# jlko/STOVE

Measured on AMD Instinct MI355X. Metric: frames/s (fwd+bwd) for 3-obj billiards 32x32 T=100, 1/2/4/8 GPU; ELBO delta vs ref, higher is better.
Workload: dtype f32 (encoder GEMMs: fp32 products as 3 sixteen-bit MFMAs on hi/lo-split operands -- half pieces forward, bf16 pieces backward -- fp32 accumulate)

## Files before the change

### stove_amd/csrc/capi.hip

```cpp
#include "../../include/stove_hip.h"
#include <algorithm>

#include "common.h"
#include <string.h>
#include <stdlib.h>
#include <math.h>
#include <atomic>
#include <type_traits>
#include "validate.h"
static_assert(stove_validate::kStoveInvalidValue == (int)hipErrorInvalidValue, "validate.h returns hipErrorInvalidValue");
#define STOVE_VALIDATE(expr)                      \
  do {                                            \
    const int v__ = stove_validate::expr;         \
    if (v__) return v__;                          \
  } while (0)
#include "spn_obj.hip"
#include "spn_obj_generic.hip"
#include "spn_bg.hip"
#include "spn_bg_generic.hip"
#include "scene.hip"
#include "scene_fused.hip"
#include "scene_colour.hip"
#include "gnn.hip"
#include "match.hip"
// ... 317 lines not shown
    inl = scene_any_inline(W_, H_);
    boxes.z = inl ? z : nullptr; boxes.n_obj = n_obj; boxes.gm = gm;
    plane = W_ * H_;
    channels = channels_;
  }
  int fork() {
    sb = scene_fork_stream(st);
    STOVE_TRY(stream_after(sb, root));
    jb.from = sb; jb.done = sb == st;
    jp.from = sp; jp.done = sp == st;
    return 0;
  }
};

template <class Obj, class Bg>
static int scene_forward(SceneCall& c, float overlap_beta, float* ll, float* parts, Obj obj_chain, Bg bg_chain) {
  int rc = c.fork();
  if (rc) return rc;
  if ((rc = obj_chain())) return rc;
  if ((rc = bg_chain())) return rc;
  STOVE_TRY(c.jb.join());
  STOVE_LAUNCH(scene_assemble_fwd_k, dim3((c.nf + 255) / 256), dim3(256), 0, c.st, c.saved + c.L.bg_out, c.saved + c.L.obj_ll,
               c.saved + c.L.ovl, c.z, ll, parts, c.n_obj, c.nf, overlap_beta, logf(overlap_beta));
  STOVE_LAUNCH_CHECK();
  return 0;
}

template <class Side, class Obj, class After>
static int scene_backward(SceneCall& c, const float* dll, float* dz, float overlap_beta, int nmax, const float* dz_bg, int bg_parts,
                          Side side_chains, Obj obj_chain, After after_finalize) {
  STOVE_LAUNCH(scene_assemble_bwd_k, dim3((c.np + 255) / 256), dim3(256), 0, c.st, dll, c.z, c.ws + c.W.d_obj, c.ws + c.W.d_ovl, c.n_obj,
               c.np, overlap_beta);
  STOVE_LAUNCH_CHECK();
  int rc = c.fork();
  if (rc) return rc;
  if ((rc = side_chains())) return rc;
  if ((rc = obj_chain())) return rc;
  STOVE_TRY(c.jb.join());
  rc = with_nmax(nmax, [&](auto n) {
    STOVE_LAUNCH((scene_finalize_bwd_k<decltype(n)::value>), dim3((c.np + 255) / 256), dim3(256), 0, c.st, dll, c.z, c.saved + c.L.obj_ll,
                 dz_bg, c.ws + c.W.dzc, dz, c.n_obj, c.np, bg_parts);
    STOVE_LAUNCH_CHECK();
    return 0;
  });
  if (rc) return rc;
  if ((rc = after_finalize())) return rc;
  c.jp.dismiss();
  return 0;
}

template <bool ANY>
static int scene_obj_fwd(const SceneCall& c, const StoveSpnTables* t, float* saved, int with_grad) {
  float* xw = saved + c.L.xw;
  int rc = with_nmax(c.n_obj, [&](auto n) { return scene_tile_fwd<decltype(n)::value, ANY>(c.frames, c.z, xw, c.n_obj, c.np, c.st, c.fm, c.gm); });
  if (rc) return rc;
  if (with_grad)
    return objspn_forward_unit(xw, t->obj_scope, t->obj_coef, t->obj_wsum, t->obj_wroot, saved + c.L.obj_ll, saved + c.L.ovl,
                               saved + c.L.obj_scratch, c.np, c.st);
  return objspn_forward(xw, t->obj_scope, t->obj_coef, t->obj_wsum, t->obj_wroot, saved + c.L.obj_ll, saved + c.L.ovl, c.np, c.st);
}
template <bool ANY>
static int scene_obj_bwd(const SceneCall& c, const StoveSpnTables* t) {
  return with_nmax(c.n_obj, [&](auto n) {
    return scene_pixtile_bwd<decltype(n)::value, ANY>(c.frames, c.z, c.saved + c.L.xw, c.saved + c.L.obj_scratch, t->obj_leaf_slot, t->obj_coef,
                                                      c.ws + c.W.d_ovl, c.ws + c.W.dzc, c.n_obj, c.np, c.st, c.fm, c.ws + c.W.d_obj, c.gm);
  });
}
static int scene_obj_tablegrads(const SceneCall& c, const StoveSpnTables* t, StoveSpnTableGrads* g, bool under = false) {
  STOVE_TRY(stream_after(c.sp, c.st));
  return objspn_backward_params(c.saved + c.L.xw, t->obj_scope, g->obj_coef, g->obj_wsum, g->obj_wroot, c.saved + c.L.obj_scratch,
                                c.ws + c.W.obj, c.ws + c.W.d_obj, c.np, c.sp, under);
}

static int scene_bg_fwd_any(const SceneCall& c, const int32_t* side, const float* coef, const float* wroot, float* saved) {
  if (!c.inl) {
    const size_t tot = (size_t)c.nf * c.plane;
    STOVE_LAUNCH(bg_mask_any_k, dim3((unsigned)((tot + 255) / 256)), dim3(256), 0, c.sb, c.z, saved + c.L.bg_aux, c.nf, c.n_obj, c.gm);
    STOVE_LAUNCH_CHECK();
  }
  return bgspn_any_forward(c.frames, c.inl ? nullptr : saved + c.L.bg_aux, side, coef, wroot, saved + c.L.bg_ell, saved + c.L.bg_out, c.nf,
                           c.channels * c.plane, c.sb, c.fm, c.boxes, c.plane);
}
static int scene_bg_bwd_any(const SceneCall& c, const int32_t* side, const float* coef, const float* wroot, const float* dll, float* g_coef,
                            float* g_wroot) {
  float* d_mask = c.ws + c.W.d_mask;
  int rc = bgspn_any_backward(c.frames, c.inl ? nullptr : c.saved + c.L.bg_aux, side, coef, wroot, c.saved + c.L.bg_ell, c.saved + c.L.bg_out,
                              dll, nullptr, d_mask, g_coef, g_wroot, c.ws + c.W.bg, c.nf, c.channels * c.plane, c.sb, c.fm, c.boxes, c.plane);
  if (rc) return rc;
  return with_nmax<false>(c.n_obj, [&](auto n) {
    STOVE_LAUNCH((bg_mask_bwd_any_k<decltype(n)::value>), dim3(c.nf), dim3(256), 0, c.sb, c.z, (const float*)d_mask, c.ws + c.W.dz_bg, c.nf,
                 c.n_obj, c.gm, c.channels);
    STOVE_LAUNCH_CHECK();
    return 0;
  });
}

}

extern "C" {

static SceneSaved scene_saved_tuned(int nf, int n_obj, bool with_grad = true) {
  return scene_saved_layout(nf, n_obj, with_grad, bgspn_fwd_ws_floats(nf), bg_cover_floats(nf, n_obj));
}
static SceneWs scene_ws_tuned(int nf, int n_obj) {
  return scene_ws_layout((size_t)nf * n_obj, nmax_of(n_obj), 0, objspn_partial_floats(), 0, bgspn_bwd_ws_floats(nf, n_obj));
}
size_t stove_scene_saved_floats(int n_frames, int n_obj) { return scene_saved_tuned(n_frames, n_obj).total; }
size_t stove_scene_fwd_floats(int n_frames, int n_obj, int with_grad) { return scene_saved_tuned(n_frames, n_obj, with_grad != 0).total; }
size_t stove_scene_bwd_ws_bytes(int n_frames, int n_obj) { return scene_ws_tuned(n_frames, n_obj).total * sizeof(float); }

size_t stove_bg_dense_floats(void) { return (size_t)kBgDenseF; }
int stove_bg_dense(const int32_t* bg_side, const float* bg_coef, float* dense, void* stream) {
  STOVE_LAUNCH(bg_dense_fwd_k, dim3((kBgDenseF + 255) / 256), dim3(256), 0, (hipStream_t)stream, bg_side, bg_coef, dense);
  STOVE_LAUNCH_CHECK();
  return 0;
}
int stove_scene_fwd(const StoveSpnTables* t, const float* frames, const float* z, int n_frames, int n_obj, int seq_frames,
                    int seq_stride, float overlap_beta, float* ll, float* parts, float* saved, void* stream) {
  return stove_scene_fwd_from(t, frames, z, n_frames, n_obj, seq_frames, seq_stride, overlap_beta, ll, parts, saved, stream, stream, 1);
}

int stove_scene_fwd_from(const StoveSpnTables* t, const float* frames, const float* z, int n_frames, int n_obj, int seq_frames,
                         int seq_stride, float overlap_beta, float* ll, float* parts, float* saved, void* stream, void* fork_from,
                         int with_grad) {
  STOVE_VALIDATE(scene_fwd(t, frames, z, n_frames, n_obj, seq_frames, seq_stride, ll, saved));
  if (n_frames == 0) return 0;
  SceneCall c(frames, z, n_frames, n_obj, stream, fork_from);
  if (frame_map(n_frames, seq_frames, seq_stride, &c.fm)) return (int)hipErrorInvalidValue;
  c.L = scene_saved_tuned(n_frames, n_obj);
  c.saved = saved;
  return scene_forward(
      c, overlap_beta, ll, parts, [&] { return scene_obj_fwd<false>(c, t, saved, with_grad); },
      [&] {
        int rc = bgspn_forward(frames, nullptr, z, n_obj, t->bg_side, t->bg_coef, t->bg_wroot, saved + c.L.bg_ell, saved + c.L.bg_out, n_frames,
                               c.sb, c.fm, t->bg_dense);
        if (rc) return rc;
        return bg_cover_tables(z, saved + c.L.bg_aux, n_frames, n_obj, c.sb);
      });
}

int stove_scene_bwd(const StoveSpnTables* t, const float* frames, const float* z, int n_frames, int n_obj, int seq_frames,
                    int seq_stride, float overlap_beta, const float* saved, const float* dll, float* dz, StoveSpnTableGrads* g,
                    void* ws_, void* stream) {
  return stove_scene_bwd_overlap(t, frames, z, n_frames, n_obj, seq_frames, seq_stride, overlap_beta, saved, dll, dz, g, ws_, stream, stream);
}

int stove_scene_bwd_overlap(const StoveSpnTables* t, const float* frames, const float* z, int n_frames, int n_obj, int seq_frames,
                            int seq_stride, float overlap_beta, const float* saved, const float* dll, float* dz,
                            StoveSpnTableGrads* g, void* ws_, void* stream, void* param_stream) {
  return stove_scene_bwd_from(t, frames, z, n_frames, n_obj, seq_frames, seq_stride, overlap_beta, saved, dll, dz, g, ws_, stream, param_stream, stream);
}

constexpr int kLateTableGradGlimpses = 16384;

int stove_scene_bwd_from(const StoveSpnTables* t, const float* frames, const float* z, int n_frames, int n_obj, int seq_frames,
                         int seq_stride, float overlap_beta, const float* saved, const float* dll, float* dz,
                         StoveSpnTableGrads* g, void* ws_, void* stream, void* param_stream, void* fork_from) {
  STOVE_VALIDATE(scene_bwd(t, frames, z, n_frames, n_obj, seq_frames, seq_stride, saved, dll, dz, g, ws_));
  if (n_frames == 0) return 0;
  SceneCall c(frames, z, n_frames, n_obj, stream, fork_from, param_stream);
  if (frame_map(n_frames, seq_frames, seq_stride, &c.fm)) return (int)hipErrorInvalidValue;
  c.L = scene_saved_tuned(n_frames, n_obj);
  c.saved = saved;
  c.W = scene_ws_tuned(n_frames, n_obj);
  c.ws = (float*)ws_;
  const bool late = c.sp != c.st && n_obj <= 4 && c.np >= kLateTableGradGlimpses;
  return scene_backward(
      c, dll, dz, overlap_beta, nmax_of(n_obj), bgspn_dz_parts(c.ws + c.W.bg, n_frames), kBgHalves,
      [&] {
        if (!late) {
          const int rc = scene_obj_tablegrads(c, t, g);
          if (rc) return rc;
        }
        return bgspn_backward(frames, nullptr, z, n_obj, t->bg_side, t->bg_coef, t->bg_wroot, saved + c.L.bg_ell, saved + c.L.bg_out, dll, nullptr,
                              nullptr, nullptr, g->bg_coef, g->bg_wroot, c.ws + c.W.bg, n_frames, c.sb, c.sp == c.st ? c.sb : c.sp, c.fm,
                              saved + c.L.bg_aux);
      },
      [&] { return scene_obj_bwd<false>(c, t); }, [&] { return late ? scene_obj_tablegrads(c, t, g, true) : 0; });
}

static ObjAnyShape obj_any_shape(int R, int G, int S, int D, int Lmax) {
  ObjAnyShape sh;
  sh.R = R; sh.G = G; sh.S = S; sh.D = D; sh.Lmax = Lmax;
  return sh;
}
size_t stove_objspn_saved_floats_any(int n, int R, int G, int S, int D, int Lmax) { return objany_saved_floats(n, obj_any_shape(R, G, S, D, Lmax)); }
size_t stove_objspn_bwd_ws_bytes_any(int n, int R, int G, int S, int D, int Lmax) { return objany_bwd_ws_floats(n, obj_any_shape(R, G, S, D, Lmax)) * sizeof(float); }
int stove_objspn_fwd_any(const float* inputs, const float* marg, const int* lscope, const float* coef, const float* wsum, const float* wroot,
                         float* saved, float* out, int n, int R, int G, int S, int D, int Lmax, void* stream) {
  return objany_forward(inputs, marg, lscope, coef, wsum, wroot, saved, out, n, obj_any_shape(R, G, S, D, Lmax), (hipStream_t)stream);
}
int stove_objspn_bwd_any(const float* inputs, const float* marg, const int* lscope, const int* slot, const float* coef, const float* wsum,
                         const float* wroot, const float* saved, const float* dout, float* d_inputs, float* d_marg, float* g_coef,
                         float* g_wsum, float* g_wroot, void* ws, int n, int R, int G, int S, int D, int Lmax, void* stream) {
  return objany_backward(inputs, marg, lscope, slot, coef, wsum, wroot, saved, dout, d_inputs, d_marg, g_coef, g_wsum, g_wroot, (float*)ws, n,
                         obj_any_shape(R, G, S, D, Lmax), (hipStream_t)stream);
}

int stove_gauss_ll_fwd(const float* x, const float* marg, float* out, int n, int d, float mean, float scale, void* stream) {
  if (n == 0) return 0;
  if (d < 1 || !(scale > 0.0f) || x == nullptr || marg == nullptr || out == nullptr) return (int)hipErrorInvalidValue;
  STOVE_LAUNCH(gauss_ll_fwd_k, dim3((n + 3) / 4), dim3(256), 0, (hipStream_t)stream, x, marg, out, n, d, mean, scale);
  STOVE_LAUNCH_CHECK();
  return 0;
}
int stove_gauss_ll_bwd(const float* x, const float* marg, const float* dout, float* dx, float* dm, int n, int d, float mean, float scale,
                       void* stream) {
  if (n == 0) return 0;
  if (d < 1 || !(scale > 0.0f) || x == nullptr || marg == nullptr || dout == nullptr) return (int)hipErrorInvalidValue;
  const size_t tot = (size_t)n * d;
  STOVE_LAUNCH(gauss_ll_bwd_k, dim3((unsigned)((tot + 255) / 256)), dim3(256), 0, (hipStream_t)stream, x, marg, dout, dx, dm, n, d, mean, scale);
  STOVE_LAUNCH_CHECK();
  return 0;
}

static SceneSaved scene_saved_any(int nf, int n_obj, int n_pix, bool with_grad, bool inline_mask = false) {
  return scene_saved_layout(nf, n_obj, with_grad, bgspn_any_saved_floats(nf, n_pix), inline_mask ? 0 : (size_t)nf * n_pix);
}
static SceneWs scene_ws_any(int nf, int n_obj, int n_pix) {
  return scene_ws_layout((size_t)nf * n_obj, nmax_of(n_obj), 0, objspn_partial_floats(), (size_t)nf * n_pix, bgspn_any_bwd_ws_floats(nf, n_pix));
}
size_t stove_scene_saved_floats_any(int n_frames, int n_obj, int n_pix, int with_grad) { return scene_saved_any(n_frames, n_obj, n_pix, with_grad != 0).total; }
size_t stove_scene_bwd_ws_bytes_any(int n_frames, int n_obj, int n_pix) { return scene_ws_any(n_frames, n_obj, n_pix).total * sizeof(float); }

int stove_scene_fwd_any(const StoveSpnTables* t, const float* frames, const float* z, int n_frames, int n_obj, int seq_frames, int seq_stride,
                        int W, int H, int align_corners, float overlap_beta, float* ll, float* parts, float* saved, void* stream, int with_grad) {
  STOVE_VALIDATE(scene_fwd(t, frames, z, n_frames, n_obj, seq_frames, seq_stride, ll, saved));
  if (n_frames == 0) return 0;
  if (W < 2 || H < 2 || n_obj < 1 || n_obj > 8) return (int)hipErrorInvalidValue;
  SceneCall c(frames, z, n_frames, n_obj, stream);
  if (frame_map(n_frames, seq_frames, seq_stride, &c.fm)) return (int)hipErrorInvalidValue;
  c.geometry(W, H, align_corners, 1);
  c.L = scene_saved_any(n_frames, n_obj, W * H, true, c.inl);
  c.saved = saved;
  return scene_forward(
      c, overlap_beta, ll, parts, [&] { return scene_obj_fwd<true>(c, t, saved, with_grad); },
      [&] { return scene_bg_fwd_any(c, t->bg_side, t->bg_coef, t->bg_wroot, saved); });
}

int stove_scene_bwd_any(const StoveSpnTables* t, const float* frames, const float* z, int n_frames, int n_obj, int seq_frames, int seq_stride,
                        int W, int H, int align_corners, float overlap_beta, const float* saved, const float* dll, float* dz,
                        StoveSpnTableGrads* g, void* ws_, void* stream, void* param_stream) {
  STOVE_VALIDATE(scene_bwd(t, frames, z, n_frames, n_obj, seq_frames, seq_stride, saved, dll, dz, g, ws_));
  if (n_frames == 0) return 0;
  if (W < 2 || H < 2 || n_obj < 1 || n_obj > 8) return (int)hipErrorInvalidValue;
  SceneCall c(frames, z, n_frames, n_obj, stream, nullptr, param_stream);
  if (frame_map(n_frames, seq_frames, seq_stride, &c.fm)) return (int)hipErrorInvalidValue;
  c.geometry(W, H, align_corners, 1);
  c.L = scene_saved_any(n_frames, n_obj, W * H, true, c.inl);
  c.saved = saved;
  c.W = scene_ws_any(n_frames, n_obj, W * H);
  c.ws = (float*)ws_;
  return scene_backward(
      c, dll, dz, overlap_beta, nmax_of(n_obj), c.ws + c.W.dz_bg, 1,
      [&] { return scene_bg_bwd_any(c, t->bg_side, t->bg_coef, t->bg_wroot, dll, g->bg_coef, g->bg_wroot); },
      [&] { return scene_obj_bwd<true>(c, t); },
      [&] { return scene_obj_tablegrads(c, t, g); });
}

static inline int nmax_ch(int n_obj) { return n_obj <= 3 ? 3 : 8; }
static SceneSaved scene_saved_ch(int nf, int n_obj, int C, int W, int H, const ObjAnyShape& sh) {
  const size_t np = (size_t)nf * n_obj;
  Layout l;
  SceneSaved s{};
  s.patches = l.take(np * sh.D);
  s.marg = l.take(np * sh.D);
  s.obj = l.take(objany_saved_floats((int)np, sh));
  scene_saved_shared(l, s, nf, np, bgspn_any_saved_floats(nf, C * W * H), scene_any_inline(W, H) ? 0 : (size_t)nf * W * H);
  s.total = l.total;
  return s;
}
static SceneWs scene_ws_ch(int nf, int n_obj, int C, int W, int H, const ObjAnyShape& sh) {
  const size_t np = (size_t)nf * n_obj, n_pix = (size_t)C * W * H;
  return scene_ws_layout(np, nmax_ch(n_obj), np * sh.D, objany_bwd_ws_floats((int)np, sh), (size_t)nf * n_pix, bgspn_any_bwd_ws_floats(nf, (int)n_pix));
}
static GlimpseGeom glimpse_geom(int pw, int ph, int align_corners) {
  GlimpseGeom g;
  g.pw = pw; g.ph = ph;
  if (align_corners) {
    g.pax = 2.0f / (ph - 1); g.pbx = -1.0f; g.pay = 2.0f / (pw - 1); g.pby = -1.0f;
  } else {
    g.pax = 2.0f / ph; g.pbx = 1.0f / ph - 1.0f; g.pay = 2.0f / pw; g.pby = 1.0f / pw - 1.0f;
  }
  return g;
}
size_t stove_scene_saved_floats_ch(int n_frames, int n_obj, int channels, int W, int H, int R, int G, int S, int D, int Lmax, int with_grad) {
  (void)with_grad;
  return scene_saved_ch(n_frames, n_obj, channels, W, H, obj_any_shape(R, G, S, D, Lmax)).total;
}
size_t stove_scene_bwd_ws_bytes_ch(int n_frames, int n_obj, int channels, int W, int H, int R, int G, int S, int D, int Lmax) {
  return scene_ws_ch(n_frames, n_obj, channels, W, H, obj_any_shape(R, G, S, D, Lmax)).total * sizeof(float);
}

int stove_scene_fwd_ch(const int32_t* lscope, const int32_t* slot, const float* coef, const float* wsum, const float* wroot, int R, int G, int S,
                       int D, int Lmax, const int32_t* bg_side, const float* bg_coef, const float* bg_wroot, size_t bg_coef_floats,
                       const float* frames, const float* z, int n_frames, int n_obj, int seq_frames, int seq_stride, int channels, int W, int H,
                       int pw, int ph, int align_corners, float overlap_beta, float* ll, float* parts, float* saved, void* stream, int with_grad) {
  (void)slot;
  (void)with_grad;
  STOVE_VALIDATE(scene_ch_fwd(lscope, coef, wsum, wroot, R, G, S, D, Lmax, bg_side, bg_coef, bg_wroot, bg_coef_floats, frames, z, n_frames, n_obj,
                              seq_frames, seq_stride, channels, W, H, pw, ph, ll, saved));
  if (n_frames == 0) return 0;
  SceneCall c(frames, z, n_frames, n_obj, stream);
  if (frame_map(n_frames, seq_frames, seq_stride, &c.fm)) return (int)hipErrorInvalidValue;
  const ObjAnyShape sh = obj_any_shape(R, G, S, D, Lmax);
  const GlimpseGeom gg = glimpse_geom(pw, ph, align_corners);
// ... 1466 lines not shown
```

### stove_amd/csrc/spn_obj.hip

```cpp
#include "common.h"

namespace stove {

template <int N>
__device__ __forceinline__ float vmax(const float (&v)[N]) {
  float m = v[0];
#pragma unroll
  for (int i = 1; i < N; ++i) m = fmaxf(m, v[i]);
  return m;
}

template <int N>
struct LaneTable {
  float v[(N + 63) / 64];
  __device__ __forceinline__ void load(const float* __restrict__ p, int lane) {
#pragma unroll
    for (int i = 0; i < (N + 63) / 64; ++i) v[i] = (i * 64 + lane < N) ? p[i * 64 + lane] : 0.0f;
  }
  __device__ __forceinline__ float at(int idx) const {
    return __int_as_float(__builtin_amdgcn_readlane(__float_as_int(v[idx >> 6]), idx & 63));
  }
};

template <int N>
// ... 475 lines not shown
  const float4 sc = wrow ? tg_scale4(scale, first_sample + 4 * (threadIdx.x & 15)) : float4{1.0f, 1.0f, 1.0f, 1.0f};
  for (int i = threadIdx.x; i < 2 * D * 16; i += NT) {
    float4 v = src[i];
    v.x *= sc.x; v.y *= sc.y; v.z *= sc.z; v.w *= sc.w;
    *reinterpret_cast<float4*>(tileP + (i >> 4) * LD + 4 * (i & 15)) = v;
  }
}

template <int R, int S, int G, int K>
__global__ __launch_bounds__(128 * R) void objspn_tablegrad_k(
    const float* __restrict__ xw, const float* __restrict__ Dscr, const float* __restrict__ Sscr, const float* __restrict__ Rscr,
    const int* __restrict__ scope, float* __restrict__ part_c, float* __restrict__ part_w, float* __restrict__ part_r,
    int n_batches, int n_chunks, const float* __restrict__ scale) {
  constexpr int D = 4 * S, LD = 68, NS = K + 2 * G;
  constexpr int TC = (3 * S + 15) / 16, TW = (G * G + 15) / 16;
  static_assert(G <= 16 && K <= 16, "one column tile");
  typedef __attribute__((ext_vector_type(4))) float f4;
  extern __shared__ __attribute__((aligned(16))) float tg_lds[];
  float* tileP = tg_lds;
  float* nodeS = tileP + 2 * D * LD;
  const int lane = lane_id(), wv = wave_id();
  const int r = wv >> 1, side = wv & 1, node = wv;
  const int rr = lane & 15, kk = lane >> 4;
  const int c = blockIdx.x;
  int c_row[2][TC], c_feat[2][TC];
#pragma unroll
  for (int l2 = 0; l2 < 2; ++l2)
#pragma unroll
    for (int t = 0; t < TC; ++t) {
      const int row = min(16 * t + rr, 3 * S - 1);
      c_feat[l2][t] = row / S;
      c_row[l2][t] = 2 * scope[(r * 4 + side * 2 + l2) * S + row % S];
    }
  int w_e1[TW], w_e2[TW];
#pragma unroll
  for (int t = 0; t < TW; ++t) {
    const int row = min(16 * t + rr, G * G - 1);
    w_e1[t] = K + row % G;
    w_e2[t] = K + G + row / G;
  }
  f4 acc_c[2][TC], acc_w[TW], acc_r;
#pragma unroll
  for (int l2 = 0; l2 < 2; ++l2)
#pragma unroll
    for (int t = 0; t < TC; ++t) acc_c[l2][t] = f4{0.0f, 0.0f, 0.0f, 0.0f};
#pragma unroll
  for (int t = 0; t < TW; ++t) acc_w[t] = f4{0.0f, 0.0f, 0.0f, 0.0f};
  acc_r = f4{0.0f, 0.0f, 0.0f, 0.0f};

  for (int b = c; b < n_batches; b += n_chunks) {
    {
      tg_stage_tile<D, LD, 128 * R>(tileP, xw + (size_t)b * (D * 2 * 64), scale, b * 64);
      const float4* ss = reinterpret_cast<const float4*>(Sscr + (size_t)(b * R * 2 + node) * NS * 64);
      float* dst = nodeS + node * NS * LD;
      for (int i = lane; i < NS * 16; i += 64) *reinterpret_cast<float4*>(dst + (i >> 4) * LD + 4 * (i & 15)) = ss[i];
    }
    __syncthreads();
#pragma unroll
    for (int l2 = 0; l2 < 2; ++l2) {
      const int L = side * 2 + l2;
      const float4* dp = reinterpret_cast<const float4*>(Dscr + (((size_t)(b * R + r) * 4 + L) * G + min(rr, G - 1)) * 64 + 16 * kk);
      const float4 d0 = dp[0], d1 = dp[1], d2 = dp[2], d3 = dp[3];
      const float dv[16] = {d0.x, d0.y, d0.z, d0.w, d1.x, d1.y, d1.z, d1.w, d2.x, d2.y, d2.z, d2.w, d3.x, d3.y, d3.z, d3.w};
#pragma unroll
      for (int t = 0; t < TC; ++t) {
        const float* xr = tileP + c_row[l2][t] * LD + 16 * kk;
        const int feat = c_feat[l2][t];
#pragma unroll
        for (int h = 0; h < 4; ++h) {
          const float4 x4 = *reinterpret_cast<const float4*>(xr + 4 * h);
          const float4 w4 = *reinterpret_cast<const float4*>(xr + LD + 4 * h);
          const float xs[4] = {x4.x, x4.y, x4.z, x4.w}, ws[4] = {w4.x, w4.y, w4.z, w4.w};
#pragma unroll
          for (int e = 0; e < 4; ++e) {
            const float wx = ws[e] * xs[e];
            const float fv = feat == 0 ? wx * xs[e] : (feat == 1 ? wx : ws[e]);
            acc_c[l2][t] = __builtin_amdgcn_mfma_f32_16x16x4f32(fv, dv[4 * h + e], acc_c[l2][t], 0, 0, 0);
          }
        }
      }
    }
    {
      const float* nb = nodeS + node * NS * LD + 16 * kk;
      const float* gp = nb + min(rr, K - 1) * LD;
      float gv[16];
#pragma unroll
      for (int h = 0; h < 4; ++h) {
        const float4 g4 = *reinterpret_cast<const float4*>(gp + 4 * h);
        const float4 s4 = tg_scale4(scale, b * 64 + 16 * kk + 4 * h);
        gv[4 * h] = g4.x * s4.x; gv[4 * h + 1] = g4.y * s4.y; gv[4 * h + 2] = g4.z * s4.z; gv[4 * h + 3] = g4.w * s4.w;
      }
#pragma unroll
      for (int t = 0; t < TW; ++t) {
        const float* e1 = nb + w_e1[t] * LD;
        const float* e2 = nb + w_e2[t] * LD;
#pragma unroll
        for (int h = 0; h < 4; ++h) {
          const float4 a4 = *reinterpret_cast<const float4*>(e1 + 4 * h);
          const float4 b4 = *reinterpret_cast<const float4*>(e2 + 4 * h);
          acc_w[t] = __builtin_amdgcn_mfma_f32_16x16x4f32(a4.x * b4.x, gv[4 * h], acc_w[t], 0, 0, 0);
          acc_w[t] = __builtin_amdgcn_mfma_f32_16x16x4f32(a4.y * b4.y, gv[4 * h + 1], acc_w[t], 0, 0, 0);
          acc_w[t] = __builtin_amdgcn_mfma_f32_16x16x4f32(a4.z * b4.z, gv[4 * h + 2], acc_w[t], 0, 0, 0);
          acc_w[t] = __builtin_amdgcn_mfma_f32_16x16x4f32(a4.w * b4.w, gv[4 * h + 3], acc_w[t], 0, 0, 0);
        }
      }
    }
    if (side == 0) {
      const float* rp = Rscr + (size_t)(b * R + r) * (1 + 2 * K) * 64 + 16 * kk;
      const float4* rho = reinterpret_cast<const float4*>(rp);
      const float4* ea = reinterpret_cast<const float4*>(rp + (1 + min(rr, K - 1)) * 64);
      const float4* eb = reinterpret_cast<const float4*>(rp + (1 + K + min(rr, K - 1)) * 64);
#pragma unroll
      for (int h = 0; h < 4; ++h) {
        const float4 q4 = rho[h], a4 = ea[h], b4 = eb[h];
        const float4 s4 = tg_scale4(scale, b * 64 + 16 * kk + 4 * h);
        acc_r = __builtin_amdgcn_mfma_f32_16x16x4f32(q4.x * s4.x * b4.x, a4.x, acc_r, 0, 0, 0);
        acc_r = __builtin_amdgcn_mfma_f32_16x16x4f32(q4.y * s4.y * b4.y, a4.y, acc_r, 0, 0, 0);
        acc_r = __builtin_amdgcn_mfma_f32_16x16x4f32(q4.z * s4.z * b4.z, a4.z, acc_r, 0, 0, 0);
        acc_r = __builtin_amdgcn_mfma_f32_16x16x4f32(q4.w * s4.w * b4.w, a4.w, acc_r, 0, 0, 0);
      }
    }
    __syncthreads();
  }
  const int col = lane & 15;
#pragma unroll
  for (int l2 = 0; l2 < 2; ++l2)
#pragma unroll
    for (int t = 0; t < TC; ++t)
#pragma unroll
      for (int e = 0; e < 4; ++e) {
        const int row = 16 * t + 4 * kk + e;
        if (row < 3 * S && col < G) {
          const int feat = row / S, i = row % S;
          part_c[((size_t)(c * R + r) * D + (side * 2 + l2) * S + i) * G * 3 + col * 3 + feat] = acc_c[l2][t][e];
        }
      }
#pragma unroll
  for (int t = 0; t < TW; ++t)
#pragma unroll
    for (int e = 0; e < 4; ++e) {
      const int row = 16 * t + 4 * kk + e;
      if (row < G * G && col < K) part_w[((size_t)(c * R * 2 + node) * G * G + row) * K + col] = acc_w[t][e];
    }
  if (side == 0) {
#pragma unroll
    for (int e = 0; e < 4; ++e) {
      const int row = 4 * kk + e;
      if (row < K && col < K) part_r[((size_t)(c * R + r) * K + row) * K + col] = acc_r[e];
    }
  }
}

template <int R, int S, int G, int K>
__global__ __launch_bounds__(256, 3) void objspn_tablegrad_under_k(
   
    const float* __restrict__ xw, const float* __restrict__ Dscr, const float* __restrict__ Sscr, const float* __restrict__ Rscr,
    const int* __restrict__ scope, float* __restrict__ part_c, float* __restrict__ part_w, float* __restrict__ part_r,
    int n_batches, int n_chunks, const float* __restrict__ scale) {
  constexpr int D = 4 * S, LD = 68, NS = K + 2 * G;
  constexpr int TC = (3 * S + 15) / 16, TW = (G * G + 15) / 16, TWH = (TW + 1) / 2;
  static_assert(G <= 16 && K <= 16, "one column tile");
  typedef __attribute__((ext_vector_type(4))) float f4;
  extern __shared__ __attribute__((aligned(16))) float tg_lds[];
  float* tileP = tg_lds;
  float* scl = tileP + 2 * D * LD;
  const int lane = lane_id(), wv = wave_id();
  int c, r;
  if ((n_chunks & 7) == 0) {
    const int xcd = blockIdx.x & 7, j = blockIdx.x >> 3;
    c = xcd * (n_chunks >> 3) + j / R;
    r = j % R;
  } else {
    c = blockIdx.x / R;
    r = blockIdx.x % R;
  }
  const int side = wv & 1, half = wv >> 1, node = 2 * r + side, L = side * 2 + half;
  const int rr = lane & 15, kk = lane >> 4;
  int c_row[TC], c_feat[TC];
#pragma unroll
  for (int t = 0; t < TC; ++t) {
    const int row = min(16 * t + rr, 3 * S - 1);
    c_feat[t] = row / S;
    c_row[t] = 2 * scope[(r * 4 + L) * S + row % S];
  }
  int w_e1[TWH], w_e2[TWH];
#pragma unroll
  for (int i = 0; i < TWH; ++i) {
    const int row = min(16 * (half * TWH + i) + rr, G * G - 1);
    w_e1[i] = K + row % G;
    w_e2[i] = K + G + row / G;
  }
  f4 acc_c[TC], acc_w[TWH], acc_r = f4{0.0f, 0.0f, 0.0f, 0.0f};
#pragma unroll
  for (int t = 0; t < TC; ++t) acc_c[t] = f4{0.0f, 0.0f, 0.0f, 0.0f};
#pragma unroll
  for (int i = 0; i < TWH; ++i) acc_w[i] = f4{0.0f, 0.0f, 0.0f, 0.0f};

  for (int b = c; b < n_batches; b += n_chunks) {
    tg_stage_tile<D, LD, 256>(tileP, xw + (size_t)b * (D * 2 * 64), scale, b * 64);
    if (threadIdx.x < 16) *reinterpret_cast<float4*>(scl + 4 * threadIdx.x) = tg_scale4(scale, b * 64 + 4 * threadIdx.x);
    __syncthreads();
    {
      const float4* dp = reinterpret_cast<const float4*>(Dscr + (((size_t)(b * R + r) * 4 + L) * G + min(rr, G - 1)) * 64 + 16 * kk);
      const float4 d0 = dp[0], d1 = dp[1], d2 = dp[2], d3 = dp[3];
      const float dv[16] = {d0.x, d0.y, d0.z, d0.w, d1.x, d1.y, d1.z, d1.w, d2.x, d2.y, d2.z, d2.w, d3.x, d3.y, d3.z, d3.w};
#pragma unroll
      for (int h = 0; h < 4; ++h) {
        float fv[TC][4];
#pragma unroll
        for (int t = 0; t < TC; ++t) {
          const float* xr = tileP + c_row[t] * LD + 16 * kk + 4 * h;
          const float4 x4 = *reinterpret_cast<const float4*>(xr);
          const float4 w4 = *reinterpret_cast<const float4*>(xr + LD);
          const float xs[4] = {x4.x, x4.y, x4.z, x4.w}, ws[4] = {w4.x, w4.y, w4.z, w4.w};
#pragma unroll
          for (int e = 0; e < 4; ++e) {
            const float wx = ws[e] * xs[e];
            fv[t][e] = c_feat[t] == 0 ? wx * xs[e] : (c_feat[t] == 1 ? wx : ws[e]);
          }
        }
#pragma unroll
        for (int e = 0; e < 4; ++e)
#pragma unroll
          for (int t = 0; t < TC; ++t) acc_c[t] = __builtin_amdgcn_mfma_f32_16x16x4f32(fv[t][e], dv[4 * h + e], acc_c[t], 0, 0, 0);
      }
    }
    {
      const float* nb = Sscr + (size_t)(b * R * 2 + node) * NS * 64 + 16 * kk;
      const float* gp = nb + min(rr, K - 1) * 64;
#pragma unroll
      for (int h = 0; h < 4; ++h) {
        const float4 g4 = *reinterpret_cast<const float4*>(gp + 4 * h);
        const float4 s4 = *reinterpret_cast<const float4*>(scl + 16 * kk + 4 * h);
        const float gv[4] = {g4.x * s4.x, g4.y * s4.y, g4.z * s4.z, g4.w * s4.w};
        float pr[TWH][4];
#pragma unroll
        for (int i = 0; i < TWH; ++i) {
          const float4 a4 = *reinterpret_cast<const float4*>(nb + w_e1[i] * 64 + 4 * h);
          const float4 b4 = *reinterpret_cast<const float4*>(nb + w_e2[i] * 64 + 4 * h);
          pr[i][0] = a4.x * b4.x; pr[i][1] = a4.y * b4.y; pr[i][2] = a4.z * b4.z; pr[i][3] = a4.w * b4.w;
        }
#pragma unroll
        for (int e = 0; e < 4; ++e)
#pragma unroll
          for (int i = 0; i < TWH; ++i)
            acc_w[i] = __builtin_amdgcn_mfma_f32_16x16x4f32(pr[i][e], gv[e], acc_w[i], 0, 0, 0);
      }
    }
    if (side == 0 && half == 1) {
      const float* rp = Rscr + (size_t)(b * R + r) * (1 + 2 * K) * 64 + 16 * kk;
      const float4* rho = reinterpret_cast<const float4*>(rp);
      const float4* ea = reinterpret_cast<const float4*>(rp + (1 + min(rr, K - 1)) * 64);
      const float4* eb = reinterpret_cast<const float4*>(rp + (1 + K + min(rr, K - 1)) * 64);
#pragma unroll
      for (int h = 0; h < 4; ++h) {
        const float4 q4 = rho[h], a4 = ea[h], b4 = eb[h];
        const float4 s4 = *reinterpret_cast<const float4*>(scl + 16 * kk + 4 * h);
        acc_r = __builtin_amdgcn_mfma_f32_16x16x4f32(q4.x * s4.x * b4.x, a4.x, acc_r, 0, 0, 0);
        acc_r = __builtin_amdgcn_mfma_f32_16x16x4f32(q4.y * s4.y * b4.y, a4.y, acc_r, 0, 0, 0);
        acc_r = __builtin_amdgcn_mfma_f32_16x16x4f32(q4.z * s4.z * b4.z, a4.z, acc_r, 0, 0, 0);
        acc_r = __builtin_amdgcn_mfma_f32_16x16x4f32(q4.w * s4.w * b4.w, a4.w, acc_r, 0, 0, 0);
      }
    }
    __syncthreads();
  }
  const int col = lane & 15;
#pragma unroll
  for (int t = 0; t < TC; ++t)
#pragma unroll
    for (int e = 0; e < 4; ++e) {
      const int row = 16 * t + 4 * kk + e;
      if (row < 3 * S && col < G) {
        const int feat = row / S, i = row % S;
        part_c[((size_t)(c * R + r) * D + L * S + i) * G * 3 + col * 3 + feat] = acc_c[t][e];
      }
    }
#pragma unroll
  for (int i = 0; i < TWH; ++i)
#pragma unroll
    for (int e = 0; e < 4; ++e) {
      const int row = 16 * (half * TWH + i) + 4 * kk + e;
      if (row < G * G && col < K) part_w[((size_t)(c * R * 2 + node) * G * G + row) * K + col] = acc_w[i][e];
    }
  if (side == 0 && half == 1) {
#pragma unroll
    for (int e = 0; e < 4; ++e) {
      const int row = 4 * kk + e;
      if (row < K && col < K) part_r[((size_t)(c * R + r) * K + row) * K + col] = acc_r[e];
    }
  }
}

__global__ void objspn_tile_from_arrays_k(const float* __restrict__ inputs, const float* __restrict__ marg,
                                          float* __restrict__ xw, int n_samples, int n_batches, int D) {
  extern __shared__ float lds[];
  const int stride = D + 1;
  for (int b = blockIdx.x; b < n_batches; b += gridDim.x) {
    for (int i = threadIdx.x; i < 64 * D; i += blockDim.x) {
      const int smp = i / D, p = i % D;
      const size_t gi = (size_t)(b * 64 + smp) * D + p;
      const bool live = (b * 64 + smp) < n_samples;
      const float x = live ? inputs[gi] : 0.0f;
      float w = 0.0f;
      if (live) w = (marg != nullptr) ? 1.0f - fminf(fmaxf(marg[gi], 0.0f), 1.0f) : 1.0f;
      lds[smp * stride + p] = x;
      lds[64 * stride + smp * stride + p] = w;
    }
    __syncthreads();
    float* tile = xw + (size_t)b * D * 2 * 64;
    for (int i = threadIdx.x; i < 64 * D * 2; i += blockDim.x) {
      const int lane = i & 63, pc = i >> 6;
      tile[i] = lds[(pc & 1) * 64 * stride + lane * stride + (pc >> 1)];
    }
    __syncthreads();
  }
}

__global__ void objspn_tile_to_arrays_k(const float* __restrict__ dxw, const float* __restrict__ marg,
                                        float* __restrict__ d_inputs, float* __restrict__ d_marg,
                                        int n_samples, int n_batches, int D) {
  extern __shared__ float lds[];
  const int stride = D + 1;
  for (int b = blockIdx.x; b < n_batches; b += gridDim.x) {
    const float* tile = dxw + (size_t)b * D * 2 * 64;
    for (int i = threadIdx.x; i < 64 * D * 2; i += blockDim.x) {
      const int lane = i & 63, pc = i >> 6;
      lds[(pc & 1) * 64 * stride + lane * stride + (pc >> 1)] = tile[i];
    }
    __syncthreads();
    for (int i = threadIdx.x; i < 64 * D; i += blockDim.x) {
      const int smp = i / D, p = i % D;
      if ((b * 64 + smp) >= n_samples) continue;
      const size_t gi = (size_t)(b * 64 + smp) * D + p;
      if (d_inputs != nullptr) d_inputs[gi] = lds[smp * stride + p];
      if (d_marg != nullptr) {
        const float m = marg[gi];
        d_marg[gi] = (m >= 0.0f && m <= 1.0f) ? -lds[64 * stride + smp * stride + p] : 0.0f;
      }
    }
    __syncthreads();
  }
}

__global__ __launch_bounds__(256) void reduce_chunks_k(const float* __restrict__ part, float* __restrict__ out, int n, int n_chunks, int accumulate,
                                                       float* __restrict__ out2 = nullptr) {
  __shared__ float red[8][32];
  const int e = threadIdx.x & 31, q = threadIdx.x >> 5;
  const int j = blockIdx.x * 32 + e;
  float s = 0.0f;
  if (j < n)
    for (int c = q; c < n_chunks; c += 8) s += part[(size_t)c * n + j];
  red[q][e] = s;
  __syncthreads();
  if (q == 0 && j < n) {
    float t = red[0][e];
#pragma unroll
    for (int k = 1; k < 8; ++k) t += red[k][e];
    out[j] = accumulate ? out[j] + t : t;
    if (out2 != nullptr) out2[j] = accumulate ? out2[j] + t : t;
  }
}

struct Reduce3 {
  const float* part[3];
  float* out[3];
  int n[3];
};
__global__ __launch_bounds__(256) void reduce_chunks3_k(Reduce3 a, int n_chunks) {
  __shared__ float red[8][32];
  const int e = threadIdx.x & 31, q = threadIdx.x >> 5;
  int blk = blockIdx.x, seg = 0;
#pragma unroll
  for (int k = 0; k < 2; ++k) {
    const int nbk = (a.n[k] + 31) / 32;
    if (seg == k && blk >= nbk) {
      blk -= nbk;
      seg = k + 1;
    }
  }
  const float* __restrict__ part = seg == 0 ? a.part[0] : (seg == 1 ? a.part[1] : a.part[2]);
  float* __restrict__ out = seg == 0 ? a.out[0] : (seg == 1 ? a.out[1] : a.out[2]);
  const int n = seg == 0 ? a.n[0] : (seg == 1 ? a.n[1] : a.n[2]);
  const int j = blk * 32 + e;
  float s = 0.0f;
  if (j < n)
    for (int c = q; c < n_chunks; c += 8) s += part[(size_t)c * n + j];
  red[q][e] = s;
  __syncthreads();
  if (q == 0 && j < n) {
    float t = red[0][e];
#pragma unroll
    for (int k = 1; k < 8; ++k) t += red[k][e];
    out[j] = t;
  }
}

}

namespace stove {

static inline int grid_for(int n_items, int cap) { return n_items < cap ? (n_items > 0 ? n_items : 1) : cap; }

int objspn_tile_from_arrays(const float* inputs, const float* marg, float* xw, int n, hipStream_t st) {
  const int nb = (n + 63) / 64;
  if (nb == 0) return 0;
  const int D = 100;
  STOVE_LAUNCH(objspn_tile_from_arrays_k, dim3(grid_for(nb, 2048)), dim3(256), 2 * 64 * (D + 1) * sizeof(float), st,
                     inputs, marg, xw, n, nb, D);
  STOVE_LAUNCH_CHECK();
  return 0;
}

int objspn_tile_to_arrays(const float* dxw, const float* marg, float* d_inputs, float* d_marg, int n, hipStream_t st) {
  const int nb = (n + 63) / 64;
  if (nb == 0) return 0;
  const int D = 100;
  STOVE_LAUNCH(objspn_tile_to_arrays_k, dim3(grid_for(nb, 2048)), dim3(256), 2 * 64 * (D + 1) * sizeof(float), st,
                     dxw, marg, d_inputs, d_marg, n, nb, D);
  STOVE_LAUNCH_CHECK();
  return 0;
}

int objspn_forward(const float* xw, const int* scope, const float* coef, const float* wsum, const float* wroot,
                   float* out, float* ovl, int n, hipStream_t st) {
  const int nb = (n + 63) / 64;
  if (nb == 0) return 0;
  STOVE_LAUNCH((objspn_fwd_k<6, 25, 10, 10>), dim3(grid_for(nb, 4096)), dim3(768), 0, st,
                     xw, scope, coef, wsum, wroot, out, ovl, n, nb);
  STOVE_LAUNCH_CHECK();
  return 0;
}

int objspn_mpe(const float* xw, const int* scope, const float* coef, const float* wsum, const float* wroot, const float* mu,
               float* out, int* pick, int n, hipStream_t st) {
  const int nb = (n + 63) / 64;
  if (nb == 0) return 0;
  STOVE_LAUNCH((objspn_mpe_k<6, 25, 10, 10>), dim3(grid_for(nb, 4096)), dim3(768), 0, st,
                     xw, scope, coef, wsum, wroot, mu, out, pick, n, nb);
  STOVE_LAUNCH_CHECK();
  return 0;
}

constexpr size_t kObjD = 6 * 4 * 10 * 64, kObjS = 12 * 30 * 64, kObjR = 6 * 21 * 64, kObjX = 100 * 2 * 64;
constexpr int kObjChunks = 256;
constexpr size_t kObjCoefN = 6 * 100 * 10 * 3, kObjWN = 12 * 100 * 10, kObjRootN = 6 * 100;

size_t objspn_scratch_floats(int n) { return (size_t)((n + 63) / 64) * (kObjD + kObjS + kObjR); }
size_t objspn_partial_floats() { return (size_t)kObjChunks * (kObjCoefN + kObjWN + kObjRootN); }
size_t objspn_bwd_ws_floats(int n) { return objspn_scratch_floats(n) + objspn_partial_floats(); }

int objspn_forward_unit(const float* xw, const int* scope, const float* coef, const float* wsum, const float* wroot,
                        float* out, float* ovl, float* scratch, int n, hipStream_t st) {
  const int nb = (n + 63) / 64;
  if (nb == 0) return 0;
  float* Dscr = scratch;
  float* Sscr = Dscr + (size_t)nb * kObjD;
  float* Rscr = Sscr + (size_t)nb * kObjS;
  STOVE_LAUNCH((objspn_fwd_unit_k<6, 25, 10, 10>), dim3(grid_for(nb, 4096)), dim3(768), 0, st,
                     xw, scope, coef, wsum, wroot, out, ovl, Dscr, Sscr, Rscr, n, nb);
  STOVE_LAUNCH_CHECK();
  return 0;
}

int objspn_backward_data(const float* xw, const int* scope, const int* leaf_slot, const float* coef, const float* wsum,
                         const float* wroot, const float* out, const float* dout, float* dxw, float* scratch, int n, hipStream_t st) {
  const int nb = (n + 63) / 64;
  if (nb == 0) return 0;
  float* Dscr = scratch;
  float* Sscr = Dscr + (size_t)nb * kObjD;
  float* Rscr = Sscr + (size_t)nb * kObjS;
  STOVE_LAUNCH((objspn_bwd_k<6, 25, 10, 10>), dim3(grid_for(nb, 4096)), dim3(768), 0, st,
                     xw, scope, coef, wsum, wroot, out, dout, Dscr, Sscr, Rscr, n, nb);
  STOVE_LAUNCH_CHECK();
  if (dxw == nullptr) return 0;
  STOVE_LAUNCH((objspn_pix_k<6, 25, 10, 8>), dim3(grid_for(nb, 4096)), dim3(512), 0, st,
                     xw, Dscr, leaf_slot, coef, dxw, nb);
  STOVE_LAUNCH_CHECK();
  return 0;
}

int objspn_backward_params(const float* xw, const int* scope, float* g_coef, float* g_wsum, float* g_wroot, const float* scratch,
                           float* partial, const float* scale, int n, hipStream_t st, bool under = false) {
  const int nb = (n + 63) / 64;
  if (nb == 0) {
    hipMemsetAsync(g_coef, 0, kObjCoefN * 4, st);
    hipMemsetAsync(g_wsum, 0, kObjWN * 4, st);
    hipMemsetAsync(g_wroot, 0, kObjRootN * 4, st);
    return 0;
  }
  const float* Dscr = scratch;
  const float* Sscr = Dscr + (size_t)nb * kObjD;
  const float* Rscr = Sscr + (size_t)nb * kObjS;
  float* pc = partial;
  float* pw = pc + (size_t)kObjChunks * kObjCoefN;
  float* pr = pw + (size_t)kObjChunks * kObjWN;
  int chunks = nb < kObjChunks ? nb : kObjChunks;
  if (under) {
    constexpr int kTgLdsU = (2 * 100 * 68 + 64) * (int)sizeof(float);
    if (chunks > kObjChunks / 6) chunks = (kObjChunks / 6) & ~7;
    int rc = (int)hipFuncSetAttribute((const void*)objspn_tablegrad_under_k<6, 25, 10, 10>, hipFuncAttributeMaxDynamicSharedMemorySize, kTgLdsU);
    if (rc) return rc;
    STOVE_LAUNCH((objspn_tablegrad_under_k<6, 25, 10, 10>), dim3(chunks * 6), dim3(256), kTgLdsU, st, xw, Dscr, Sscr, Rscr, scope, pc, pw, pr, nb, chunks, scale);
    STOVE_LAUNCH_CHECK();
  } else {
    constexpr int kTgLds = (2 * 100 * 68 + 12 * 30 * 68) * (int)sizeof(float);
    int rc = (int)hipFuncSetAttribute((const void*)objspn_tablegrad_k<6, 25, 10, 10>, hipFuncAttributeMaxDynamicSharedMemorySize, kTgLds);
    if (rc) return rc;
    STOVE_LAUNCH((objspn_tablegrad_k<6, 25, 10, 10>), dim3(chunks), dim3(768), kTgLds, st, xw, Dscr, Sscr, Rscr, scope, pc, pw, pr, nb, chunks, scale);
    STOVE_LAUNCH_CHECK();
  }
  Reduce3 r3;
  r3.part[0] = pc; r3.part[1] = pw; r3.part[2] = pr;
  r3.out[0] = g_coef; r3.out[1] = g_wsum; r3.out[2] = g_wroot;
  r3.n[0] = (int)kObjCoefN; r3.n[1] = (int)kObjWN; r3.n[2] = (int)kObjRootN;
  STOVE_LAUNCH(reduce_chunks3_k, dim3((kObjCoefN + 31) / 32 + (kObjWN + 31) / 32 + (kObjRootN + 31) / 32), dim3(256), 0, st, r3, chunks);
  STOVE_LAUNCH_CHECK();
  return 0;
}

int objspn_backward(const float* xw, const int* scope, const int* leaf_slot, const float* coef, const float* wsum,
                    const float* wroot, const float* out, const float* dout, float* dxw,
                    float* g_coef, float* g_wsum, float* g_wroot, float* ws, int n, hipStream_t st) {
  int rc = objspn_backward_data(xw, scope, leaf_slot, coef, wsum, wroot, out, dout, dxw, ws, n, st);
  if (rc) return rc;
  return objspn_backward_params(xw, scope, g_coef, g_wsum, g_wroot, ws, ws + objspn_scratch_floats(n), nullptr, n, st);
}

}
```

Baseline: 9.316 million.

## Software-pipeline global loads in object-SPN under-kernel table gradient

Restructures objspn_tablegrad_under_k so the next batch's xw tile, scale and leaf gradients are loaded into registers during the current batch's MFMA work, and per-h sum/root scratch loads are issued one step ahead of their use. The occupancy hint drops from 3 to 2 waves per SIMD, with a VGPR cap of 100 to make room for the prefetch registers. The goal is to hide global-memory latency behind compute. The cost is lower occupancy and higher register pressure. A static_assert is added to check that the kernel's LDS still fits next to the concurrent dyn_loop kernel.

```diff
diff --git a/stove_amd/csrc/capi.hip b/stove_amd/csrc/capi.hip
--- a/stove_amd/csrc/capi.hip
+++ b/stove_amd/csrc/capi.hip
@@ -493,6 +493,8 @@
 }
 
 constexpr int kLateTableGradGlimpses = 16384;
+static_assert(kTgLdsU + smb_lds_floats<4>() * (int)sizeof(float) + 64 * kSmWaves * (int)sizeof(float) + 512 <= 160 * 1024,
+              "objspn_tablegrad_under_k no longer fits into the LDS that dyn_loop_bwd_small_k<4, ..> leaves free");
 
 int stove_scene_bwd_from(const StoveSpnTables* t, const float* frames, const float* z, int n_frames, int n_obj, int seq_frames,
                          int seq_stride, float overlap_beta, const float* saved, const float* dll, float* dz,
diff --git a/stove_amd/csrc/spn_obj.hip b/stove_amd/csrc/spn_obj.hip
--- a/stove_amd/csrc/spn_obj.hip
+++ b/stove_amd/csrc/spn_obj.hip
@@ -651,8 +651,7 @@
 }
 
 template <int R, int S, int G, int K>
-__global__ __launch_bounds__(256, 3) void objspn_tablegrad_under_k(
-   
+__global__ __launch_bounds__(256, 2) __attribute__((amdgpu_num_vgpr(100))) void objspn_tablegrad_under_k(
     const float* __restrict__ xw, const float* __restrict__ Dscr, const float* __restrict__ Sscr, const float* __restrict__ Rscr,
     const int* __restrict__ scope, float* __restrict__ part_c, float* __restrict__ part_w, float* __restrict__ part_r,
     int n_batches, int n_chunks, const float* __restrict__ scale) {
@@ -682,12 +681,13 @@
     c_feat[t] = row / S;
     c_row[t] = 2 * scope[(r * 4 + L) * S + row % S];
   }
-  int w_e1[TWH], w_e2[TWH];
+  const int o_kk = 16 * kk, o_g = min(rr, K - 1) * 64 + 16 * kk;
+  int o_e1[TWH], o_e2[TWH];
 #pragma unroll
   for (int i = 0; i < TWH; ++i) {
     const int row = min(16 * (half * TWH + i) + rr, G * G - 1);
-    w_e1[i] = K + row % G;
-    w_e2[i] = K + G + row / G;
+    o_e1[i] = (K + row % G) * 64 + 16 * kk;
+    o_e2[i] = (K + G + row / G) * 64 + 16 * kk;
   }
   f4 acc_c[TC], acc_w[TWH], acc_r = f4{0.0f, 0.0f, 0.0f, 0.0f};
 #pragma unroll
@@ -695,13 +695,62 @@
 #pragma unroll
   for (int i = 0; i < TWH; ++i) acc_w[i] = f4{0.0f, 0.0f, 0.0f, 0.0f};
 
+  constexpr int NT4 = 2 * D * 16, TI = (NT4 + 255) / 256;
+  const bool wrow = ((threadIdx.x >> 4) & 1) != 0;
+  const bool root = side == 0 && half == 1;
+  float* const tile_dst = tileP + (threadIdx.x >> 4) * LD + 4 * (threadIdx.x & 15);
+  float4 tv[TI], tsc, dn[4];
+  auto tile_fetch = [&](int b) {
+    const float4* src = reinterpret_cast<const float4*>(xw + (size_t)b * (D * 2 * 64));
+#pragma unroll
+    for (int j = 0; j < TI; ++j)
+      if (256 * (j + 1) <= NT4 || (int)threadIdx.x + 256 * j < NT4) tv[j] = src[threadIdx.x + 256 * j];
+    tsc = wrow ? tg_scale4(scale, b * 64 + 4 * (threadIdx.x & 15)) : float4{1.0f, 1.0f, 1.0f, 1.0f};
+  };
+  auto tile_store = [&]() {
+#pragma unroll
+    for (int j = 0; j < TI; ++j)
+      if (256 * (j + 1) <= NT4 || (int)threadIdx.x + 256 * j < NT4) {
+        float4 v = tv[j];
+        v.x *= tsc.x; v.y *= tsc.y; v.z *= tsc.z; v.w *= tsc.w;
+        *reinterpret_cast<float4*>(tile_dst + j * 16 * LD) = v;
+      }
+    if ((threadIdx.x >> 4) == 1) *reinterpret_cast<float4*>(scl + 4 * (threadIdx.x & 15)) = tsc;
+  };
+  auto leaf_fetch = [&](int b) {
+    const float* dp = Dscr + (size_t)__builtin_amdgcn_readfirstlane((b * R + r) * 4 + L) * (G * 64);
+#pragma unroll
+    for (int q = 0; q < 4; ++q) dn[q] = *reinterpret_cast<const float4*>(dp + o_g + 4 * q);
+  };
+  struct SumIn { float4 g, a[TWH], b[TWH], q, ea, eb; };
+  auto sum_fetch = [&](int b, int h, SumIn& s) {
+    const float* nb = Sscr + (size_t)__builtin_amdgcn_readfirstlane(b * R * 2 + node) * (NS * 64) + 4 * h;
+    s.g = *reinterpret_cast<const float4*>(nb + o_g);
+#pragma unroll
+    for (int i = 0; i < TWH; ++i) {
+      s.a[i] = *reinterpret_cast<const float4*>(nb + o_e1[i]);
+      s.b[i] = *reinterpret_cast<const float4*>(nb + o_e2[i]);
+    }
+    if (root) {
+      const float* rp = Rscr + (size_t)__builtin_amdgcn_readfirstlane(b * R + r) * ((1 + 2 * K) * 64) + 4 * h;
+      s.q = *reinterpret_cast<const float4*>(rp + o_kk);
+      s.ea = *reinterpret_cast<const float4*>(rp + 64 + o_g);
+      s.eb = *reinterpret_cast<const float4*>(rp + (1 + K) * 64 + o_g);
+    }
+  };
+
+  if (c < n_batches) {
+    tile_fetch(c);
+    leaf_fetch(c);
+  }
   for (int b = c; b < n_batches; b += n_chunks) {
-    tg_stage_tile<D, LD, 256>(tileP, xw + (size_t)b * (D * 2 * 64), scale, b * 64);
-    if (threadIdx.x < 16) *reinterpret_cast<float4*>(scl + 4 * threadIdx.x) = tg_scale4(scale, b * 64 + 4 * threadIdx.x);
-    __syncthreads();
+    const int bn = b + n_chunks < n_batches ? b + n_chunks : b;
+    tile_store();
+    const float4 d0 = dn[0], d1 = dn[1], d2 = dn[2], d3 = dn[3];
+    __syncthreads();
+    SumIn cur;
+    sum_fetch(b, 0, cur);
     {
-      const float4* dp = reinterpret_cast<const float4*>(Dscr + (((size_t)(b * R + r) * 4 + L) * G + min(rr, G - 1)) * 64 + 16 * kk);
-      const float4 d0 = dp[0], d1 = dp[1], d2 = dp[2], d3 = dp[3];
       const float dv[16] = {d0.x, d0.y, d0.z, d0.w, d1.x, d1.y, d1.z, d1.w, d2.x, d2.y, d2.z, d2.w, d3.x, d3.y, d3.z, d3.w};
 #pragma unroll
       for (int h = 0; h < 4; ++h) {
@@ -724,41 +773,35 @@
           for (int t = 0; t < TC; ++t) acc_c[t] = __builtin_amdgcn_mfma_f32_16x16x4f32(fv[t][e], dv[4 * h + e], acc_c[t], 0, 0, 0);
       }
     }
-    {
-      const float* nb = Sscr + (size_t)(b * R * 2 + node) * NS * 64 + 16 * kk;
-      const float* gp = nb + min(rr, K - 1) * 64;
-#pragma unroll
-      for (int h = 0; h < 4; ++h) {
-        const float4 g4 = *reinterpret_cast<const float4*>(gp + 4 * h);
-        const float4 s4 = *reinterpret_cast<const float4*>(scl + 16 * kk + 4 * h);
-        const float gv[4] = {g4.x * s4.x, g4.y * s4.y, g4.z * s4.z, g4.w * s4.w};
-        float pr[TWH][4];
-#pragma unroll
-        for (int i = 0; i < TWH; ++i) {
-          const float4 a4 = *reinterpret_cast<const float4*>(nb + w_e1[i] * 64 + 4 * h);
-          const float4 b4 = *reinterpret_cast<const float4*>(nb + w_e2[i] * 64 + 4 * h);
-          pr[i][0] = a4.x * b4.x; pr[i][1] = a4.y * b4.y; pr[i][2] = a4.z * b4.z; pr[i][3] = a4.w * b4.w;
-        }
-#pragma unroll
-        for (int e = 0; e < 4; ++e)
-#pragma unroll
-          for (int i = 0; i < TWH; ++i)
-            acc_w[i] = __builtin_amdgcn_mfma_f32_16x16x4f32(pr[i][e], gv[e], acc_w[i], 0, 0, 0);
-      }
-    }
-    if (side == 0 && half == 1) {
-      const float* rp = Rscr + (size_t)(b * R + r) * (1 + 2 * K) * 64 + 16 * kk;
-      const float4* rho = reinterpret_cast<const float4*>(rp);
-      const float4* ea = reinterpret_cast<const float4*>(rp + (1 + min(rr, K - 1)) * 64);
-      const float4* eb = reinterpret_cast<const float4*>(rp + (1 + K + min(rr, K - 1)) * 64);
-#pragma unroll
-      for (int h = 0; h < 4; ++h) {
-        const float4 q4 = rho[h], a4 = ea[h], b4 = eb[h];
-        const float4 s4 = *reinterpret_cast<const float4*>(scl + 16 * kk + 4 * h);
-        acc_r = __builtin_amdgcn_mfma_f32_16x16x4f32(q4.x * s4.x * b4.x, a4.x, acc_r, 0, 0, 0);
-        acc_r = __builtin_amdgcn_mfma_f32_16x16x4f32(q4.y * s4.y * b4.y, a4.y, acc_r, 0, 0, 0);
-        acc_r = __builtin_amdgcn_mfma_f32_16x16x4f32(q4.z * s4.z * b4.z, a4.z, acc_r, 0, 0, 0);
-        acc_r = __builtin_amdgcn_mfma_f32_16x16x4f32(q4.w * s4.w * b4.w, a4.w, acc_r, 0, 0, 0);
+    __builtin_amdgcn_sched_barrier(0);
+#pragma unroll
+    for (int h = 0; h < 4; ++h) {
+      const float4 s4 = *reinterpret_cast<const float4*>(scl + 16 * kk + 4 * h);
+      const float gv[4] = {cur.g.x * s4.x, cur.g.y * s4.y, cur.g.z * s4.z, cur.g.w * s4.w};
+      float pr[TWH][4];
+#pragma unroll
+      for (int i = 0; i < TWH; ++i) {
+        pr[i][0] = cur.a[i].x * cur.b[i].x; pr[i][1] = cur.a[i].y * cur.b[i].y; pr[i][2] = cur.a[i].z * cur.b[i].z; pr[i][3] = cur.a[i].w * cur.b[i].w;
+      }
+      float ra[4], rb[4];
+      if (root) {
+        ra[0] = cur.q.x * s4.x * cur.eb.x; ra[1] = cur.q.y * s4.y * cur.eb.y; ra[2] = cur.q.z * s4.z * cur.eb.z; ra[3] = cur.q.w * s4.w * cur.eb.w;
+        rb[0] = cur.ea.x; rb[1] = cur.ea.y; rb[2] = cur.ea.z; rb[3] = cur.ea.w;
+      }
+      if (h < 3) {
+        sum_fetch(b, h + 1, cur);
+      } else {
+        tile_fetch(bn);
+        leaf_fetch(bn);
+      }
+#pragma unroll
+      for (int e = 0; e < 4; ++e)
+#pragma unroll
+        for (int i = 0; i < TWH; ++i)
+          acc_w[i] = __builtin_amdgcn_mfma_f32_16x16x4f32(pr[i][e], gv[e], acc_w[i], 0, 0, 0);
+      if (root) {
+#pragma unroll
+        for (int e = 0; e < 4; ++e) acc_r = __builtin_amdgcn_mfma_f32_16x16x4f32(ra[e], rb[e], acc_r, 0, 0, 0);
       }
     }
     __syncthreads();
@@ -978,6 +1021,8 @@
   return 0;
 }
 
+constexpr int kTgLdsU = (2 * 100 * 68 + 64) * (int)sizeof(float);
+
 int objspn_backward_params(const float* xw, const int* scope, float* g_coef, float* g_wsum, float* g_wroot, const float* scratch,
                            float* partial, const float* scale, int n, hipStream_t st, bool under = false) {
   const int nb = (n + 63) / 64;
@@ -995,7 +1040,6 @@
   float* pr = pw + (size_t)kObjChunks * kObjWN;
   int chunks = nb < kObjChunks ? nb : kObjChunks;
   if (under) {
-    constexpr int kTgLdsU = (2 * 100 * 68 + 64) * (int)sizeof(float);
     if (chunks > kObjChunks / 6) chunks = (kObjChunks / 6) & ~7;
     int rc = (int)hipFuncSetAttribute((const void*)objspn_tablegrad_under_k<6, 25, 10, 10>, hipFuncAttributeMaxDynamicSharedMemorySize, kTgLdsU);
     if (rc) return rc;
```

Measured after the change: 9.433 million, median of 6. 1.01x the previous value.
